# adthoms/dcora

Hardware: AMD Instinct MI355X
Metric: RBCD iterations/sec, sphere2500 5-agent split (higher is better)
Workload: dtype f64

## Files before the change

dcora_amd/capi.py:

```python
import ctypes as C
import os
import subprocess

import numpy as np

_HERE = os.path.dirname(os.path.abspath(__file__))
LIB_PATH = os.path.join(_HERE, "lib", "libdcora_hip.so")
HEADER_PATH = os.path.join(os.path.dirname(_HERE), "include", "dcora_hip.h")


class DcoraError(RuntimeError):
    def __init__(self, status, msg):
        super().__init__("dcora status %d: %s" % (status, msg))
        self.status = status


class Dims(C.Structure):
    _fields_ = [("r", C.c_int), ("d", C.c_int), ("n", C.c_int), ("l", C.c_int), ("b", C.c_int), ("layout", C.c_int)]


LAYOUT_AUTO, LAYOUT_SE, LAYOUT_RA = 0, 1, 2


class ROptParams(C.Structure):
# ... 167 lines not shown
    "dcora_exchange_create_ra": (C.c_int, [_vp, C.c_char_p, C.POINTER(_vp)]),
    "dcora_exchange_info": (C.c_int, [_vp, _dp]),
    "dcora_exchange_link_report": (C.c_int, [_vp, _dp]),
    "dcora_exchange_post": (C.c_int, [_vp, _ip, C.c_int]),
    "dcora_exchange_wait": (C.c_int, [_vp, _ip, C.c_int]),
    "dcora_exchange_evaluate": (C.c_int, [_vp, _PD, _PD, _vp, _PI]),
    "dcora_exchange_rbcd_iterate": (C.c_int, [_vp, C.c_int, _PD, _PD, _vp, _PI]),
    "dcora_exchange_rbcd_tick": (C.c_int, [_vp, _ip, C.c_int, C.c_int]),
    "dcora_exchange_run_coloured": (C.c_int, [_vp, C.c_int, C.c_double, _PI, _vp, _vp]),
    "dcora_exchange_set_X": (C.c_int, [_vp, _dp]),
    "dcora_exchange_gather_X": (C.c_int, [_vp, _dp]),
    "dcora_exchange_barrier": (C.c_int, [_vp]),
    "dcora_exchange_all_ready": (C.c_int, [_vp, C.c_int, _PI]),
    "dcora_exchange_update_weights": (C.c_int, [_vp, C.c_int, _vp]),
    "dcora_exchange_set_weights": (C.c_int, [_vp, _dp]),
    "dcora_exchange_get_weights": (C.c_int, [_vp, _dp]),
    "dcora_exchange_certify": (C.c_int, [_vp, C.c_int, _vp, _vp, _vp, C.c_double, _PI, _PD, _PD, _dp,
                                         C.POINTER(C.c_longlong), _PI]),
    "dcora_exchange_host_selftest": (C.c_int, [C.c_char_p, C.c_int, C.c_int, C.c_int, C.c_int, _PD]),
    "dcora_exchange_host_selftest_team": (C.c_int, [C.c_char_p, C.c_int, C.c_int, C.c_int, C.c_int, C.c_int, _PD]),
    "dcora_exchange_team_enable": (C.c_int, [_vp, C.POINTER(TeamParams)]),
    "dcora_exchange_agent_status": (C.c_int, [_vp, C.c_int, C.POINTER(AgentStatus), _PI]),
    "dcora_exchange_loop_closure_stats": (C.c_int, [_vp, C.c_int, _ip]),
    "dcora_exchange_should_terminate": (C.c_int, [_vp, _PI]),
    "dcora_exchange_should_update_weights": (C.c_int, [_vp, _PI]),
    "dcora_exchange_team_info": (C.c_int, [_vp, _ip]),
    "dcora_exchange_run_team": (C.c_int, [_vp, _PI, _vp, _vp, _vp, _vp, _PI, _PI]),
    "dcora_debug_exchange_leave_stale": (C.c_int, [C.c_char_p, C.c_int, C.c_int]),
    "dcora_debug_exchange_probe_fault": (C.c_int, [C.c_int]),
    "dcora_cert_prepare": (C.c_int, [C.POINTER(Dims), _ip, _ip, C.c_int, C.c_int]),
    "dcora_debug_tcg_run_fault": (C.c_int, [C.c_int]),
    "dcora_debug_tcg_run_fault_at": (C.c_int, [C.c_int, C.c_int]),
    "dcora_debug_wg_sums": (C.c_int, [C.c_int, _dp, _dp]),
    "dcora_problem_solver_info": (C.c_int, [_vp, _dp]),
    "dcora_ra_rbcd_create": (C.c_int, [_vp, C.POINTER(RbcdOptions), C.POINTER(_vp)]),
    "dcora_ra_rbcd_destroy": (C.c_int, [_vp]),
    "dcora_ra_rbcd_info": (C.c_int, [_vp, _PI, _vp]),
    "dcora_ra_rbcd_set_X": (C.c_int, [_vp, _dp]),
    "dcora_ra_rbcd_get_X": (C.c_int, [_vp, _dp]),
    "dcora_ra_rbcd_certify": (C.c_int, [_vp, C.c_double, _PI, _PD, _PD, _vp, C.POINTER(C.c_longlong), _vp]),
    "dcora_ra_rbcd_iterate": (C.c_int, [_vp, C.c_int, _PD, _PD, _vp, _PI]),
    "dcora_ra_rbcd_evaluate": (C.c_int, [_vp, _PD, _PD, _vp, _PI]),
    "dcora_ra_rbcd_run": (C.c_int, [_vp, C.c_int, C.c_double, _PI, _vp, _vp, _vp]),
    "dcora_ra_rbcd_iterate_set": (C.c_int, [_vp, _ip, C.c_int, C.c_int]),
    "dcora_ra_rbcd_set_acceleration": (C.c_int, [_vp, C.c_int]),
    "dcora_ra_rbcd_agent_colours": (C.c_int, [_vp, _ip, _PI]),
    "dcora_ra_rbcd_run_coloured": (C.c_int, [_vp, C.c_int, C.c_double, _PI, _vp, _vp]),
    "dcora_ra_rbcd_last_result": (C.c_int, [_vp, C.POINTER(ROptResult)]),
    "dcora_problem_time_qapply": (C.c_int, [_vp, C.c_int, _PD, _PD]),
    "dcora_problem_time_qapply_rotating": (C.c_int, [C.POINTER(_vp), C.c_int, C.c_int, _PD]),
    "dcora_problem_qapply_info": (C.c_int, [_vp, _dp]),
    "dcora_problem_time_precond": (C.c_int, [_vp, C.c_int, _PD, _PD]),
    "dcora_problem_precond_info": (C.c_int, [_vp, _dp]),
    "dcora_precond_cache_info": (C.c_int, [_dp]),
    "dcora_precond_cache_clear": (C.c_int, []),
    "dcora_robust_params_default": (None, [C.POINTER(RobustParams)]),
    "dcora_robust_weights": (C.c_int, [C.POINTER(RobustParams), C.c_int, C.c_int, _dp, _dp]),
    "dcora_chi2inv": (C.c_int, [C.c_double, C.c_int, _PD]),
    "dcora_robust_error_threshold_at_quantile": (C.c_int, [C.c_double, C.c_int, _PD]),
    "dcora_robust_single_rotation_averaging": (C.c_int, [C.c_int, C.c_int, _dp, _vp, C.c_double, _dp, _ip]),
    "dcora_robust_single_pose_averaging": (C.c_int, [C.c_int, C.c_int, _dp, _dp, _vp, _vp, C.c_double, _dp, _dp, _ip]),
    "dcora_agent_neighbor_transforms": (C.c_int, [C.c_int, C.c_int, _ip, _dp, _dp, _dp, _dp, _dp]),
    "dcora_agent_robust_neighbor_transform": (C.c_int, [C.c_int, C.c_int, _dp, C.c_int, C.c_int, _dp, _PI, _PI]),
    "dcora_log_trajectory": (C.c_int, [C.c_char_p, C.c_int, C.c_int, _dp]),
    "dcora_fixed_stiefel_variable": (C.c_int, [C.c_int, C.c_int, _dp]),
    "dcora_agent_initialize_in_global_frame": (C.c_int, [C.POINTER(Dims), _dp, _dp, _dp, _dp]),
# ... 49 lines not shown
```

dcora_amd/csrc/capi.hip:

```cpp
#include <cstdio>
#include <cstring>
#include <new>

#include "../../include/dcora_hip.h"
#include "cert.h"
#include "device_chol.h"
#include "device_problem.h"
#include "host_graph.h"
#include "host_threads.h"
#include "ra_rbcd.h"
#include "rbcd.h"
#include "precond_cache.h"
#include "exchange.h"
#include "host_robust.h"
#include "robust.h"
#include "round.h"

namespace dcora {
const std::string &get_last_error();
}
using namespace dcora;

struct dcora_problem_s {
  DeviceProblem p;
// ... 249 lines not shown
  });
}

int dcora_problem_solver_info(dcora_problem_t p, double *info) {
  return abi_call({p, info}, [&]() -> int {
    const DeviceProblem &P = p->p;
    info[0] = !P.use_pc() ? 0 : (P.tcg_run_ok ? 2 : 1);
    return DCORA_OK;
  });
}
int dcora_debug_tcg_run_fault(int runs) {
  g_tcg_run_fault_skip.store(0);
  g_tcg_run_fault.store(runs < 0 ? 0 : runs);
  return DCORA_OK;
}
int dcora_debug_tcg_run_fault_at(int skip, int runs) {
  g_tcg_run_fault_skip.store(skip < 0 ? 0 : skip);
  g_tcg_run_fault.store(runs < 0 ? 0 : runs);
  return DCORA_OK;
}
int dcora_debug_wg_sums(int nv, const double *in, double *out) {
  return abi_call({in, out}, [&]() -> int {
    if (no_device()) return DCORA_ERR_NO_DEVICE;
    if (nv != 33 && nv != 41 && nv != 49) return bad("dcora_debug_wg_sums: nv is 33, 41 or 49 (8 r + 1 at r = 4, 5, 6)");
    const size_t nin = (size_t)nv * 256, nout = (size_t)2 * nv * 17;
    DevBuf<double> I, O;
    DCORA_HIP(I.alloc(nin));
    DCORA_HIP(O.alloc(nout));
    DCORA_HIP(hipMemcpy(I.p, in, nin * sizeof(double), hipMemcpyHostToDevice));
    DCORA_HIP(hipMemset(O.p, 0, nout * sizeof(double)));
    if (launch_debug_wg_sums(nullptr, nv, I.p, O.p) < 0) return bad("dcora_debug_wg_sums: the launch failed");
    DCORA_HIP(hipDeviceSynchronize());
    DCORA_HIP(hipMemcpy(out, O.p, nout * sizeof(double), hipMemcpyDeviceToHost));
    return DCORA_OK;
  });
}
int dcora_problem_time_precond(dcora_problem_t p, int reps, double *avg_ms, double *bytes) {
  return abi_call({p, avg_ms, bytes}, [&] { return p->p.time_precond(reps, avg_ms, bytes); });
}
int dcora_problem_precond_info(dcora_problem_t p, double *info) {
  return abi_call({p, info}, [&]() -> int {
    const DeviceProblem &P = p->p;
    info[0] = !P.has_precond ? 0 : (P.sparse_precond ? 2 : 1);
    info[1] = !P.has_precond ? 0 : (P.sparse_precond ? P.sp.launches() : 1);
    info[2] = (double)P.precond_nnzL;
    info[3] = P.precond_setup_ms;
    info[4] = !P.has_precond ? 0 : (P.sparse_precond ? P.sp.weights_per_apply : (double)P.m.k * P.m.k);
    return DCORA_OK;
  });
}

int dcora_debug_sparse_weights_digest(dcora_problem_t p, double *out4) {
  return abi_call({p, out4}, [&]() -> int {
    const DeviceProblem &P = p->p;
    if (!P.sparse_precond || !P.sp.im) return bad("the problem has no sparse preconditioner");
    const DevBuf<double> &v = P.sp.im->vals;
    std::vector<double> h(v.n);
    DCORA_HIP(hipSetDevice(P.device));
    DCORA_HIP(hipMemcpy(h.data(), v.p, v.n * sizeof(double), hipMemcpyDeviceToHost));
    long double s0 = 0, s1 = 0, s2 = 0;
    for (size_t i = 0; i < h.size(); ++i) {
      s0 += h[i];
      s1 += std::fabs(h[i]);
      s2 += h[i] * (double)(i % 97 + 1);
    }
    out4[0] = (double)h.size();
// ... 1551 lines not shown
```

dcora_amd/csrc/fused_run.hip:

```cpp
#include <algorithm>
#include <atomic>
#include <cstdio>

#include "kernels.h"
#include "tcg_rules.h"
#include "pose_group.h"
#include "fused_pc.h"

namespace dcora {

namespace {

__device__ __forceinline__ int wg_sums_logical_lane(int p) { return ((p >> 5) & 1) | ((p >> 3) & 2) | ((p & 15) << 2); }
template <bool HALF32>
__device__ __forceinline__ double wg_sums_swap_add(double x, double y) {
  typedef unsigned u2 __attribute__((ext_vector_type(2)));
  u2 lo, hi;
  if constexpr (HALF32) {
    lo = __builtin_amdgcn_permlane32_swap((unsigned)__double2loint(x), (unsigned)__double2loint(y), false, false);
    hi = __builtin_amdgcn_permlane32_swap((unsigned)__double2hiint(x), (unsigned)__double2hiint(y), false, false);
  } else {
    lo = __builtin_amdgcn_permlane16_swap((unsigned)__double2loint(x), (unsigned)__double2loint(y), false, false);
    hi = __builtin_amdgcn_permlane16_swap((unsigned)__double2hiint(x), (unsigned)__double2hiint(y), false, false);
  }
  return __hiloint2double((int)hi[0], (int)lo[0]) + __hiloint2double((int)hi[1], (int)lo[1]);
}
template <int NV>
__device__ __forceinline__ void wg_row_sums(const double (&v)[NV], double (*sP)[4 * kPcNW], int wave, int lane) {
  constexpr int N1 = (NV + 1) / 2, N2 = (N1 + 1) / 2;
  double a[N1], b[N2];
#pragma unroll
  for (int j = 0; j < N1; ++j) a[j] = wg_sums_swap_add<true>(v[2 * j], 2 * j + 1 < NV ? v[2 * j + 1] : 0.0);
#pragma unroll
  for (int j = 0; j < N2; ++j) {
    double s = wg_sums_swap_add<false>(a[2 * j], 2 * j + 1 < N1 ? a[2 * j + 1] : 0.0);
    s += dpp_move<0xB1>(s);
    s += dpp_move<0x4E>(s);
    b[j] = s;
  }
  if ((lane & 3) == 0) {
    const int sub = ((lane >> 3) & 2) | (lane >> 5), slot = wave * 4 + ((lane >> 2) & 3);
#pragma unroll
    for (int j = 0; j < N2; ++j)
      if (4 * j + sub < NV) sP[4 * j + sub][slot] = b[j];
  }
}

constexpr int kRunShards = 32, kRunCopies = 64, kRunStride = 32;
constexpr int kRunSyncWords = (kRunShards + 1 + kRunCopies + 1) * kRunStride;
constexpr int kRunQCap = 1024;
struct TcgRunArgs {
  ManiDesc m;
  int ldm;
  const double *Minv;
  CsrDev Q;
  Buf2 grad, X, S;
  double *d0, *d1, *Hd, *eta, *Heta, *z, *p1r, *p3, *pC;
  unsigned *sync;
  SolverCtl *ctl;
  HostFlags *hf;
  int seq, pbA;
  int fault;
#ifdef DCORA_RUN_STAMPS
  long long *stamps;
#endif
};
#ifdef DCORA_RUN_STAMPS
#define RUN_STAMP(i)                                                            \
  do {                                                                          \
    __builtin_amdgcn_sched_barrier(0);                                          \
    if (a.stamps && blockIdx.x == 0 && threadIdx.x == 0 && (i) < 64) a.stamps[(i)] = wall_clock64(); \
    __builtin_amdgcn_sched_barrier(0);                                          \
  } while (0)
#else
#define RUN_STAMP(i) \
  do {                \
  } while (0)
#endif
constexpr int kRunStamp0 = 4, kRunStampsPerIter = 10;
__device__ __forceinline__ double ld_coh(const double *p) {
  return __hip_atomic_load(p, __ATOMIC_RELAXED, __HIP_MEMORY_SCOPE_AGENT);
}
__device__ __forceinline__ void st_coh(double *p, double v) {
  __hip_atomic_store(p, v, __ATOMIC_RELAXED, __HIP_MEMORY_SCOPE_AGENT);
}
__device__ __forceinline__ double2 pc_ld16_coh(__amdgpu_buffer_rsrc_t rs, unsigned voff, unsigned soff) {
  const pc_v4u v = __builtin_amdgcn_raw_buffer_load_b128(rs, voff, soff, 16);
  return __builtin_bit_cast(double2, v);
}
constexpr unsigned kRunAbortBit = 0x80000000u;
__device__ __forceinline__ bool run_grid_step(unsigned *sync, unsigned step, int *s_ok) {
  __builtin_amdgcn_s_waitcnt(0);
  __syncthreads();
  if (threadIdx.x == 0) {
    unsigned *shard = sync, *top = sync + kRunShards * kRunStride, *done = top + kRunStride,
             *abort_w = done + kRunCopies * kRunStride;
    const int i = blockIdx.x, G = gridDim.x, sh = i % kRunShards;
    const unsigned in_shard = (unsigned)((G - sh + kRunShards - 1) / kRunShards), want = step + 1;
    const unsigned shards_used = (unsigned)(G < kRunShards ? G : kRunShards);
    const unsigned a = __hip_atomic_fetch_add(shard + sh * kRunStride, 1u, __ATOMIC_RELAXED, __HIP_MEMORY_SCOPE_AGENT);
    if (a + 1 == want * in_shard) {
      const unsigned b = __hip_atomic_fetch_add(top, 1u, __ATOMIC_RELAXED, __HIP_MEMORY_SCOPE_AGENT);
      if (!(b & kRunAbortBit) && b + 1 == want * shards_used)
        for (int c = 0; c < kRunCopies; ++c)
          __hip_atomic_store(done + c * kRunStride, want, __ATOMIC_RELAXED, __HIP_MEMORY_SCOPE_AGENT);
    }
    long long t0 = wall_clock64();
    const unsigned *p = done + (i % kRunCopies) * kRunStride;
    int ok = 1;
    unsigned spins = 0;
    while (__hip_atomic_load(p, __ATOMIC_RELAXED, __HIP_MEMORY_SCOPE_AGENT) < want) {
      __builtin_amdgcn_s_sleep(1);
      if ((++spins & 63u) == 0) {
        if (__hip_atomic_load(abort_w, __ATOMIC_RELAXED, __HIP_MEMORY_SCOPE_AGENT) != 0u) {
          ok = 0;
          break;
        }
        if (wall_clock64() - t0 > 200000) {
          unsigned cur = __hip_atomic_load(top, __ATOMIC_RELAXED, __HIP_MEMORY_SCOPE_AGENT);
          bool gave_up = false;
          for (;;) {
            if (cur & kRunAbortBit) {
              gave_up = true;
              break;
            }
            if (cur >= want * shards_used) break;
            if (__hip_atomic_compare_exchange_strong(top, &cur, cur | kRunAbortBit, __ATOMIC_RELAXED, __ATOMIC_RELAXED,
                                                     __HIP_MEMORY_SCOPE_AGENT)) {
              gave_up = true;
              break;
            }
          }
          if (gave_up) {
            __hip_atomic_store(abort_w, 1u, __ATOMIC_RELAXED, __HIP_MEMORY_SCOPE_AGENT);
            ok = 0;
            break;
          }
          t0 = wall_clock64();
        }
      }
    }
    *s_ok = ok;
  }
  __syncthreads();
  return *s_ok != 0;
}

template <int D, int R, int NS>
__global__ __launch_bounds__(kPcBlock) void k_tcg_run(TcgRunArgs a) {
  constexpr int DH = D + 1, PB = 2, NR = PB * DH, RM = R;
  extern __shared__ __align__(16) double s_img[];
  double *const s_res = s_img;
  __shared__ double s_P[NR * RM + 1][4 * kPcNW];
  __shared__ double s_Z[NR * RM + 1], s_R[NR * RM], s_W[NR * RM], s_D[NR * RM], s_H[NR * RM];
  __shared__ double s_red[16];
  __shared__ int s_ci[kRunQCap];
  __shared__ double s_v[kRunQCap];
  __shared__ int s_ok;
  SolverCtl *ctl = a.ctl;
  const int seq = a.seq;
  RUN_STAMP(0);
  const int st_o = ctl->outer_done_stamp, cur = ctl->cur & 1;
  if (seq > st_o) return;
  const double c_Delta = ctl->Delta, c_ngf = ctl->ngf;
  const int c_max_inner = ctl->max_inner;
  const ManiDesc m = a.m;
  constexpr int r = R;
  const int k = m.k, ldm = a.ldm;
  const int pose0 = blockIdx.x * PB;
  const int npose = min(PB, m.n - pose0);
  const int j0 = pose0 * DH, nrow = npose * DH;
  const int wave = threadIdx.x >> 6, lane = threadIdx.x & 63;
  const int wave_u = __builtin_amdgcn_readfirstlane(wave);
  const int e = threadIdx.x;
  const bool own = e < nrow * r;
  const size_t oown = (size_t)j0 * r + e;
  const int lc = e / r, t = e - lc * r;
  const int g = threadIdx.x >> 3, tt = threadIdx.x & (GW - 1);
  const bool pact = (g < npose) && (tt < r);
  const size_t o = (size_t)(pose0 + min(g, npose - 1)) * DH * r;
  const double *__restrict__ grad = a.grad.p[cur];
  const double *__restrict__ X = a.X.p[cur];
  const unsigned vec_bytes = (unsigned)((size_t)r * k * sizeof(double));
  const __amdgpu_buffer_rsrc_t rs_g = __builtin_amdgcn_make_buffer_rsrc(const_cast<double *>(grad), 0, vec_bytes, 0x00020000);
  const __amdgpu_buffer_rsrc_t rs_h = __builtin_amdgcn_make_buffer_rsrc(a.Hd, 0, vec_bytes, 0x00020000);
// ... 18 lines not shown
  for (int i = threadIdx.x; i < pend - pbeg; i += kPcBlock) {
    s_ci[i] = a.Q.ci[pbeg + i];
    s_v[i] = a.Q.v[pbeg + i];
  }
  const int myb = own ? a.Q.rp[j0 + lc] - pbeg : 0, mye = own ? a.Q.rp[j0 + lc + 1] - pbeg : 0;
  Row<D> Y;
  ld_row<D>(X + o, r, tt, pact, Y);
  double S[D][D];
  {
    const double *__restrict__ Sblk = a.S.p[cur];
#pragma unroll
    for (int aa = 0; aa < D; ++aa)
#pragma unroll
      for (int b = 0; b < D; ++b) S[aa][b] = (g < npose) ? Sblk[(size_t)(pose0 + g) * D * D + aa + b * D] : 0.0;
  }
  double o_r = own ? grad[oown] : 0.0, o_eta = 0, o_Heta = 0, o_d = 0, o_h = 0;
  const int cpad = ((k + 127) / 128) * 128;
  const long Nc = (long)k * r;
  const int npair = (int)((Nc + 1) >> 1);
  const int nstep = cpad / 128;
  double zr = 0, dPd = 0, ePe = 0, ePd = 0, alpha = 0, ePen = 0;
  const double n0 = c_ngf;
  int status = TR_MAXITER, iters_done = 0;
  unsigned gstep = 0;
  double acc[NR * RM + 1];
  double nrm2 = 0;
  auto product = [&](int sb) {
#pragma unroll
    for (int i = 0; i < NR * RM; ++i) acc[i] = 0;
#pragma unroll
    for (int u = 0; u < NS; ++u) {
      const int sidx = wave_u + kPcNW * u;
      if (sidx < nstep) {
        const double2 *__restrict__ xs = reinterpret_cast<const double2 *>(s_img) + (size_t)(sidx * 64 + llane) * r;
        double x[2 * RM];
#pragma unroll
        for (int tq = 0; tq < RM; ++tq) {
          const double2 xx = xs[tq];
          x[2 * tq] = xx.x;
          x[2 * tq + 1] = xx.y;
        }
#pragma unroll
        for (int tq = 0; tq < RM; ++tq)
#pragma unroll
          for (int q = 0; q < NR; ++q)
            acc[q * RM + tq] = fma(x[tq], mreg[u][q].x, fma(x[r + tq], mreg[u][q].y, acc[q * RM + tq]));
      }
    }
    RUN_STAMP(sb);
#ifdef DCORA_RUN_BUTTERFLY_SUMS
    acc[NR * RM] = nrm2;
#pragma unroll
    for (int i = 0; i <= NR * RM; ++i) {
      const double v = row16_sum_dpp(acc[i]);
      if ((lane & 15) == 0) s_P[i][wave * 4 + (lane >> 4)] = v;
    }
#else
    acc[NR * RM] = __shfl(nrm2, llane);
    wg_row_sums<NR * RM + 1>(acc, s_P, wave, lane);
#endif
    RUN_STAMP(sb + 1);
    __syncthreads();
    if ((int)threadIdx.x <= NR * RM) {
      double v = 0;
#pragma unroll
      for (int w = 0; w < 4 * kPcNW; ++w) v += s_P[threadIdx.x][w];
      s_Z[threadIdx.x] = v;
// ... 40 lines not shown
      const double gr = grad[oown];
      a0 = o_eta * gr;
      a1 = o_eta * o_Heta;
      s_R[lc * RM + t] = o_eta;
    }
    __syncthreads();
    if (wave == 0) {
      Row<D> Yn = Y;
#pragma unroll
      for (int aa = 0; aa < DH; ++aa) Yn.e[aa] += 1.0 * (pact ? s_R[(g * DH + aa) * RM + tt] : 0.0);
      row_qf<D>(Yn);
      st_row<D>(a.X.p[cur ^ 1] + o, r, tt, pact, Yn);
    }
    const double t0 = block_sum(a0, s_red);
    const double t1 = block_sum(a1, s_red);
    if (threadIdx.x == 0) {
      a.pC[2 * blockIdx.x] = t0;
      a.pC[2 * blockIdx.x + 1] = t1;
    }
  };
  auto give_up = [&]() {
    if (threadIdx.x == 0) {
      ctl->outer_done_stamp = seq - 1;
      host_store(&a.hf->tcg_abort_seq, seq);
    }
  };
#pragma unroll
  for (int u = 0; u < kPcSB; ++u) {
    const int i = u * kPcBlock + (int)threadIdx.x;
    if (i < npair) {
      const double2 x = xg[u];
      nrm2 = fma(x.x, x.x, nrm2);
      nrm2 = fma(x.y, x.y, nrm2);
      reinterpret_cast<double2 *>(s_res)[i] = x;
    }
  }
  for (long i = 2L * npair + threadIdx.x; i < (long)cpad * r; i += kPcBlock) s_res[i] = 0.0;
  if (own) s_R[lc * RM + t] = o_r;
  __syncthreads();
  RUN_STAMP(1);
  product(64);
  project_z();
  RUN_STAMP(2);
  if (c_max_inner <= 0) {
    status = TR_MAXITER;
    finish();
    return;
  }
  if (a.fault && blockIdx.x == 0) return;
  if (!run_grid_step(a.sync, gstep++, &s_ok)) return give_up();
  RUN_STAMP(3);
  for (int iter = 0;; ++iter) {
    const int par = iter & 1;
    [[maybe_unused]] const int sb0 = kRunStamp0 + kRunStampsPerIter * iter;
    double *__restrict__ d_new = par ? a.d1 : a.d0;
    const double *__restrict__ d_old = par ? a.d0 : a.d1;
    {
      constexpr int kRunGB = 24;
      double ga[kRunGB], gz[kRunGB];
      double z_own = 0;
      if (own) {
        z_own = ld_coh(a.z + oown);
#pragma unroll
        for (int q = 0; q < kRunGB; ++q) {
          const bool ok = myb + q < mye;
          const size_t oo = ok ? (size_t)s_ci[myb + q] * r + t : 0;
          gz[q] = ld_coh(a.z + oo);
          ga[q] = (iter > 0) ? ld_coh(d_old + oo) : 0.0;
        }
      }
// ... 32 lines not shown
          }
#pragma unroll
          for (int q = 0; q < 8; ++q) accw += w8[q] * (beta * a8[q] - b8[q]);
        }
        dn = (iter > 0) ? beta * o_d - z_own : -z_own;
        st_coh(d_new + oown, dn);
        o_d = dn;
        s_W[e] = accw;
        s_D[e] = dn;
      }
      __syncthreads();
      if (wave == 0) {
        Row<D> V, W;
#pragma unroll
        for (int aa = 0; aa < DH; ++aa) {
          W.e[aa] = pact ? s_W[(g * DH + aa) * r + tt] : 0.0;
          V.e[aa] = pact ? s_D[(g * DH + aa) * r + tt] : 0.0;
        }
        row_sub_AS<D>(W, V, S);
        row_tangent<D>(Y, W);
        if (pact)
#pragma unroll
          for (int aa = 0; aa < DH; ++aa) {
            st_coh(a.Hd + o + aa * r + tt, W.e[aa]);
            s_H[(g * DH + aa) * r + tt] = W.e[aa];
          }
        double dacc = 0;
#pragma unroll
        for (int aa = 0; aa < DH; ++aa) dacc += V.e[aa] * W.e[aa];
        if (!pact) dacc = 0;
        const double rs = row16_sum_dpp(dacc);
        if (lane == 0) st_coh(a.p1r + blockIdx.x, rs);
      }
      __syncthreads();
      if (own) o_h = s_H[e];
    }
    RUN_STAMP(sb0 + 1);
    if (!run_grid_step(a.sync, gstep++, &s_ok)) return give_up();
    RUN_STAMP(sb0 + 2);
    double2 xh[kPcSB];
#pragma unroll
    for (int u = 0; u < kPcSB; ++u) xh[u] = pc_ld16_coh(rs_h, voff_t, (unsigned)u * kPcBlock * 16u);
    double d_Hd;
    {
      const int rows_per = a.pbA / 2, nrows = gridDim.x, nblk = (nrows + rows_per - 1) / rows_per;
      double part = 0;
      if (lane < nblk) {
        const int b0 = lane * rows_per;
        double wsum[4] = {0, 0, 0, 0};
#pragma unroll
        for (int w = 0; w < 4; ++w) {
          double rs4[4];
#pragma unroll
          for (int q = 0; q < 4; ++q) {
            const int ri = w * 4 + q;
            rs4[q] = (ri < rows_per && b0 + ri < nrows) ? ld_coh(a.p1r + b0 + ri) : 0.0;
          }
          wsum[w] = (rs4[0] + rs4[1]) + (rs4[2] + rs4[3]);
        }
        double tsum = 0;
#pragma unroll
        for (int w = 0; w < 4; ++w) tsum += wsum[w];
        part = tsum;
      }
      d_Hd = wave_sum(part);
    }
    const double c_zr = zr, c_dPd = dPd, c_ePe = ePe, c_ePd = ePd;
    alpha = tcg_alpha(c_zr, d_Hd);
    const double e_Pe_new = tcg_e_Pe_new(alpha, c_dPd, c_ePe, c_ePd);
    const bool boundary = tcg_boundary(d_Hd, e_Pe_new, c_Delta);
    const double step = boundary ? tcg_tau(c_dPd, c_ePe, c_ePd, c_Delta) : alpha;
    ePen = e_Pe_new;
    if (own) {
      o_eta = o_eta + step * o_d;
      o_Heta = o_Heta + step * o_h;
    }
    if (boundary) {
      status = tcg_boundary_status(d_Hd);
      iters_done = iter + 1;
      finish();
      return;
    }
    if (own) {
      const double rr = fma(alpha, o_h, o_r);
      o_r = rr;
      s_R[lc * RM + t] = rr;
    }
    RUN_STAMP(sb0 + 3);
    nrm2 = 0;
#pragma unroll
    for (int u = 0; u < kPcSB; ++u) {
      const int i = u * kPcBlock + (int)threadIdx.x;
      if (i < npair) {
        double2 x = reinterpret_cast<double2 *>(s_res)[i];
        x.x = fma(alpha, xh[u].x, x.x);
        x.y = fma(alpha, xh[u].y, x.y);
        nrm2 = fma(x.x, x.x, nrm2);
        nrm2 = fma(x.y, x.y, nrm2);
        reinterpret_cast<double2 *>(s_res)[i] = x;
      }
    }
    __syncthreads();
    RUN_STAMP(sb0 + 4);
    product(sb0 + 5);
    {
      if (tcg_residual_done(sqrt(s_Z[NR * RM]), n0)) {
        status = tcg_residual_status(n0);
        iters_done = iter + 1;
        finish();
        return;
      }
    }
    project_z();
    if (iter + 1 >= c_max_inner) {
      iters_done = iter + 1;
      finish();
      return;
    }
    RUN_STAMP(sb0 + 8);
    if (!run_grid_step(a.sync, gstep++, &s_ok)) return give_up();
    RUN_STAMP(sb0 + 9);
  }
}

template <int NV>
__global__ __launch_bounds__(kPcBlock) void k_debug_wg_sums(const double *__restrict__ in, double *__restrict__ out) {
  __shared__ double s_P[NV][4 * kPcNW];
  const int wave = threadIdx.x >> 6, lane = threadIdx.x & 63;
  double v[NV];
#pragma unroll
  for (int form = 0; form < 2; ++form) {
    const int src = wave * 64 + (form == 0 ? wg_sums_logical_lane(lane) : lane);
#pragma unroll
    for (int i = 0; i < NV; ++i) v[i] = in[(size_t)i * kPcBlock + src];
    if (form == 0) {
      wg_row_sums<NV>(v, s_P, wave, lane);
    } else {
#pragma unroll
      for (int i = 0; i < NV; ++i) {
        const double s = row16_sum_dpp(v[i]);
        if ((lane & 15) == 0) s_P[i][wave * 4 + (lane >> 4)] = s;
      }
    }
    __syncthreads();
    double *__restrict__ o = out + (size_t)form * NV * (4 * kPcNW + 1);
    if ((int)threadIdx.x < NV) {
      double t = 0;
#pragma unroll
      for (int w = 0; w < 4 * kPcNW; ++w) {
        t += s_P[threadIdx.x][w];
        o[threadIdx.x * 4 * kPcNW + w] = s_P[threadIdx.x][w];
      }
      o[NV * 4 * kPcNW + threadIdx.x] = t;
    }
    __syncthreads();
  }
}

}

constexpr int kRunNS = 4;
int tcg_run_sync_words() { return kRunSyncWords; }
std::atomic<int> g_tcg_run_fault{0};
std::atomic<int> g_tcg_run_fault_skip{0};
int tcg_run_max_rows_nnz(const ManiDesc &m, const int *rp) {
  const int dh = m.d + 1;
  int worst = 0;
  for (int p0 = 0; p0 < m.n; p0 += 2) {
    const int j0 = p0 * dh, j1 = std::min(m.n, p0 + 2) * dh;
    worst = std::max(worst, rp[j1] - rp[j0]);
  }
  return worst;
}
bool tcg_run_supported(const ManiDesc &m, int ldm, int cus, int max_rows_nnz) {
  if (!m.se || m.d != 3 || m.r < 4 || m.r > 6) return false;
  if (fused_pb(m.r, m.d + 1) % 2 != 0) return false;
  if (!fused_pc_preferred(m, ldm) || fused_pc_pb(m) != 2) return false;
  const int grid = (m.n + 1) / 2;
  if (grid > cus || grid > 256) return false;
  if (m.k > kRunNS * kPcNW * 128) return false;
  const int rows_per = fused_pb(m.r, m.d + 1) / 2;
  if ((grid + rows_per - 1) / rows_per > 64) return false;
  return max_rows_nnz <= kRunQCap;
}
template <int R>
static int tcg_run_launch(hipStream_t st, const TcgRunArgs &a) {
  static LdsGrant grant;
  const int cpad = ((a.m.k + 127) / 128) * 128;
  const size_t lds = (size_t)cpad * R * sizeof(double);
  if (!grant.granted(reinterpret_cast<const void *>(&k_tcg_run<3, R, kRunNS>), lds, 40 * 1024)) return -1;
  const int grid = (a.m.n + 1) / 2;
  hipLaunchKernelGGL((k_tcg_run<3, R, kRunNS>), dim3(grid), dim3(kPcBlock), lds, st, a);
  if (hipGetLastError() != hipSuccess) return -1;
  return grid;
}
int launch_tcg_run(hipStream_t st, const TcgOperands &o, int seq) {
  count_launch();
  int fault = 0;
  bool skipped = false;
  for (int sk = g_tcg_run_fault_skip.load(); sk > 0;)
    if (g_tcg_run_fault_skip.compare_exchange_weak(sk, sk - 1)) {
      skipped = true;
      break;
    }
  for (int left = skipped ? 0 : g_tcg_run_fault.load(); left > 0;)
    if (g_tcg_run_fault.compare_exchange_weak(left, left - 1)) {
      fault = 1;
      break;
    }
  const ManiDesc &m = o.m;
  TcgRunArgs a{m, o.ldm, o.Minv, o.Q, o.grad, o.X, o.S, o.d[0], o.d[1], o.Hd, o.eta, o.Heta, o.z, o.p1, o.p3, o.pC,
               o.sync, o.ctl, o.hf, seq, fused_pb(m.r, m.d + 1), fault};
#ifdef DCORA_RUN_STAMPS
  {
    static long long *buf = nullptr;
    if (!buf) (void)hipHostMalloc((void **)&buf, 64 * sizeof(long long), hipHostMallocMapped);
    static int count = 0;
    if (buf && count > 0) {
      static double acc[64];
      static int n = 0;
      long long s0 = buf[0];
      constexpr int kShown = kRunStamp0 + 4 * kRunStampsPerIter;
      if (buf[3] > s0 && buf[kShown - 1] > 0) {
        for (int i = 0; i < kShown; ++i) acc[i] += (double)(buf[i] - s0) * 0.01;
        ++n;
      }
      for (int i = 0; i < 64; ++i) buf[i] = 0;
      if (n == 500) {
        fprintf(stderr, "k_tcg_run stamps (us from start, workgroup 0, mean of %d runs that went past their fourth iteration):", n);
        for (int i = 0; i < kShown; ++i) fprintf(stderr, " %.2f", acc[i] / n);
        fprintf(stderr, "\n");
        n = -1000000;
      }
    }
    ++count;
    a.stamps = buf;
  }
#endif
  if (m.r == 4) return tcg_run_launch<4>(st, a);
  if (m.r == 5) return tcg_run_launch<5>(st, a);
  if (m.r == 6) return tcg_run_launch<6>(st, a);
  return -1;
}
int launch_debug_wg_sums(hipStream_t st, int nv, const double *in, double *out) {
  if (nv == 33) hipLaunchKernelGGL((k_debug_wg_sums<33>), dim3(1), dim3(kPcBlock), 0, st, in, out);
  else if (nv == 41) hipLaunchKernelGGL((k_debug_wg_sums<41>), dim3(1), dim3(kPcBlock), 0, st, in, out);
  else if (nv == 49) hipLaunchKernelGGL((k_debug_wg_sums<49>), dim3(1), dim3(kPcBlock), 0, st, in, out);
  else return -1;
  return hipGetLastError() == hipSuccess ? 0 : -1;
}

}
```

dcora_amd/csrc/kernels.h:

```cpp
#pragma once
#include <hip/hip_runtime.h>

#include <atomic>
#include <climits>
#include <vector>

#include "exchange_slots.h"

namespace dcora {

constexpr int kMaxPartials = 1024;
constexpr int kBsrMaxGrid = 4096;
constexpr int kBlock = 256;
constexpr int kSpmmTile = 1536;

enum class Factor : int { Stiefel, Sphere, Euclid };
struct ManiItem {
  Factor kind;
  int col;
  int idx;
};
struct ManiDesc {
  int r, d, n, l, b, k, se;
  __host__ __device__ int rot_col(int i) const { return se ? i * (d + 1) : i * d; }
// ... 174 lines not shown
int fused_pose_blocks(const ManiDesc &m);
int fused_nsplit(const ManiDesc &m);
int fused_precond_grid(const ManiDesc &m);
int fused_update_grid(const ManiDesc &m);
struct TcgOperands {
  ManiDesc m{};
  int ldm = 0;
  const double *Minv = nullptr;
  CsrDev Q;
  BsrDev Qb;
  bool has_bsr = false;
  Buf2 grad{}, X{}, S{};
  double *d[2] = {nullptr, nullptr}, *r[2] = {nullptr, nullptr};
  double *Hd = nullptr, *eta = nullptr, *Heta = nullptr, *z = nullptr;
  double *Zpart = nullptr;
  double *W = nullptr;
  double *p1 = nullptr, *p2 = nullptr, *p3 = nullptr, *pC = nullptr;
  SolverCtl *ctl = nullptr;
  HostFlags *hf = nullptr;
  SpFold sf;
  unsigned *sync = nullptr;
  double *res_new(int iter, int first) const { return first ? r[0] : r[(iter & 1) ^ 1]; }
};
int launch_fused_hess(hipStream_t st, const TcgOperands &o, int seq, int iter, int np3);
void launch_fused_precond(hipStream_t st, const TcgOperands &o, int seq, int iter, int first, int np1);
int fused_pc_blocks(const ManiDesc &m);
bool tcg_run_supported(const ManiDesc &m, int ldm, int cus, int max_rows_nnz);
int tcg_run_sync_words();
extern std::atomic<int> g_tcg_run_fault;
extern std::atomic<int> g_tcg_run_fault_skip;
int tcg_run_max_rows_nnz(const ManiDesc &m, const int *rowptr);
int launch_tcg_run(hipStream_t st, const TcgOperands &o, int seq);
int launch_debug_wg_sums(hipStream_t st, int nv, const double *in, double *out);
bool fused_pc_preferred(const ManiDesc &m, int ldm);
bool fused_pc_ready(const ManiDesc &m, int ldm);
int launch_fused_pc(hipStream_t st, const TcgOperands &o, int seq, int iter, int first, int np1, bool retract);
enum class FinishZ {
  slices,
  keep_raw,
  from_raw
};
void launch_fused_finish(hipStream_t st, const TcgOperands &o, int seq, int iter, int first, int np2,
                         FinishZ zsrc = FinishZ::slices);
int launch_fused_grad_bsr(hipStream_t st, int r, int d, const BsrDev &A, Buf2 X, const double *G, Buf2 EG, Buf2 RG, Buf2 S,
                          int sel, double *pA, double *pB, double *posenorm, Gate g,
                          const int *agent_start = nullptr, int agents = 0, int *wg_per_agent = nullptr);
int launch_fused_grad(hipStream_t st, const ManiDesc &m, const CsrDev &Q, Buf2 X, const double *G, Buf2 EG, Buf2 RG,
                      Buf2 Sblk, int sel, double *pA, double *pB, double *posenorm, Gate g,
                      const GradRide *ride = nullptr);
int launch_g_rgrad(hipStream_t st, const ManiDesc &m, Buf2 X, Buf2 EG, Buf2 RG, Buf2 Sblk, int sel, double *partials,
                   double *posenorm, Gate g);
void launch_ctl_init(hipStream_t st, SolverCtl *c, double tol, double Delta, double maxDelta, int max_outer,
                     int stop_on_accept, int max_inner);
void launch_eval_finish(hipStream_t st, int R, const int *pose_start, const double *posenorm, const double *pA,
                        int npA, EvalOut *out_dev, int seq, double *split_scratch = nullptr, int nposes = 0,
                        const double *agent_partials = nullptr, int wg_per_agent = 0);
int eval_split_doubles();
struct RelChangeSet {
  int count;
  int agent[kMaxAgents];
};
void launch_rel_change(hipStream_t st, int r, int d, const double *X, const double *XPrev, const int *pose_start,
                       const RelChangeSet &set, double *out);
struct RelChangePublish {
  ShmStatus *slots;
  int R;
// ... 81 lines not shown
```

dcora_amd/csrc/pose_group.h:

```cpp
#pragma once
#include "kernels.h"

namespace dcora {

namespace {

constexpr int GW = 8;

__device__ __forceinline__ double f_partial4_load(const double *__restrict__ p, int np) {
  const int l = (int)(threadIdx.x & 63u);
  const double a = (l < np) ? p[l] : 0.0, b = (l + 64 < np) ? p[l + 64] : 0.0;
  const double c = (l + 128 < np) ? p[l + 128] : 0.0, d = (l + 192 < np) ? p[l + 192] : 0.0;
  return (a + b) + (c + d);
}
__device__ __forceinline__ int f_partial_index(int np) { return np <= 64 ? (int)(threadIdx.x & 63u) : (int)threadIdx.x; }
__device__ __forceinline__ double f_partial_total(double v, int np, double *sm) {
  return np <= 64 ? wave_sum(v) : block_sum(v, sm);
}
__device__ __forceinline__ double grp_sum(double v) {
  asm volatile("" : "+v"(v));
  v += dpp_move<0xB1>(v);
  asm volatile("" : "+v"(v));
  v += dpp_move<0x4E>(v);
  asm volatile("" : "+v"(v));
// ... 159 lines not shown
          B.e[p] = cs * x - sn * y;
          B.e[q] = sn * x + cs * y;
#pragma unroll
          for (int i = 0; i < D; ++i) {
            const double vx = Vm[p][i], vy = Vm[q][i];
            Vm[p][i] = cs * vx - sn * vy;
            Vm[q][i] = sn * vx + cs * vy;
          }
        }
      }
    settled = settled || off < 1e-15;
    if (__all(settled)) break;
  }
  double u[D];
#pragma unroll
  for (int j = 0; j < D; ++j) {
    const double nn = grp_sum(B.e[j] * B.e[j]);
    u[j] = B.e[j] * (nn > 0 ? 1.0 / sqrt(nn) : 0.0);
  }
  if (jacobi)
#pragma unroll
    for (int c = 0; c < D; ++c) {
      double s = 0;
#pragma unroll
      for (int j = 0; j < D; ++j) s += u[j] * Vm[j][c];
      A.e[c] = s;
    }
}

constexpr int kHessTile = 1536;
constexpr int kPosesPerBlock = kBlock / GW;
constexpr int kBsrTile = 160;

__host__ __device__ inline int fused_pb(int r, int dh) {
  const int pb = kBlock / (dh * r);
  return pb > kPosesPerBlock ? kPosesPerBlock : pb;
}

#define DCORA_LAUNCH_D(KERNEL, d, grid, st, ...)                                                 \
  do {                                                                                           \
    if ((d) == 3) hipLaunchKernelGGL(KERNEL<3>, dim3(grid), dim3(kBlock), 0, st, __VA_ARGS__);   \
    else hipLaunchKernelGGL(KERNEL<2>, dim3(grid), dim3(kBlock), 0, st, __VA_ARGS__);            \
  } while (0)

}

}
```

include/dcora_hip.h:

```cpp
#ifndef DCORA_HIP_H_
#define DCORA_HIP_H_

#ifdef __cplusplus
extern "C" {
#endif

typedef enum {
  DCORA_OK = 0,
  DCORA_ERR_BAD_ARG = 1,
  DCORA_ERR_NO_DEVICE = 2,
  DCORA_ERR_HIP = 3,
  DCORA_ERR_NOT_PD = 4,
  DCORA_ERR_NO_CONVERGENCE = 5,
  DCORA_ERR_NO_PRECONDITIONER = 6,
  DCORA_ERR_IO = 7,
  DCORA_ERR_UNSUPPORTED = 8,
  DCORA_ERR_EXCHANGE_LINK = 9
} dcora_status;

const char *dcora_status_string(int status);
const char *dcora_last_error(void);
int dcora_device_count(void);

enum {
// ... 14 lines not shown
  int method;
  int verbose;
  double gradnorm_tol;
  double RGD_stepsize;
  int RGD_use_preconditioner;
  int RTR_iterations;
  int RTR_tCG_iterations;
  double RTR_initial_radius;
} dcora_ropt_params;
void dcora_ropt_params_default(dcora_ropt_params *p);

typedef struct {
  int success;
  double fInit, gradNormInit, fOpt, gradNormOpt, elapsedMs;
  int tCGStatus;
  int outer_iterations, inner_iterations, accepted_steps;
} dcora_ropt_result;

typedef struct dcora_problem_s *dcora_problem_t;

int dcora_problem_create(const dcora_dims *dims, const int *rowptr, const int *colidx, const double *vals,
                         const double *G, double precond_reg, int device, dcora_problem_t *out);
int dcora_problem_destroy(dcora_problem_t p);
int dcora_problem_set_linear_term(dcora_problem_t p, const double *G);
int dcora_problem_cost(dcora_problem_t p, const double *X, double *f);
int dcora_problem_eucgrad(dcora_problem_t p, const double *X, double *out);
int dcora_problem_riegrad(dcora_problem_t p, const double *X, double *out, double *norm);
int dcora_problem_hessvec(dcora_problem_t p, const double *X, const double *V, double *out);
int dcora_debug_hessvec_solver_form(dcora_problem_t p, const double *X, const double *V, double *out, double *dots);
int dcora_problem_solver_info(dcora_problem_t p, double *info);
int dcora_debug_tcg_run_fault(int runs);
int dcora_debug_tcg_run_fault_at(int skip, int runs);
int dcora_debug_wg_sums(int nv, const double *in, double *out);
int dcora_problem_precondition(dcora_problem_t p, const double *X, const double *V, double *out);
int dcora_problem_retract(dcora_problem_t p, const double *X, const double *V, double *out);
int dcora_problem_tangent_project(dcora_problem_t p, const double *X, const double *V, double *out);
int dcora_problem_escape_saddle(dcora_problem_t p, const double *Xopt, double theta, const double *v,
                                double gradient_tolerance, double preconditioned_gradient_tolerance,
                                int is_second_order, double *Xout, int *success);
int dcora_manifold_project(const dcora_dims *dims, const double *M, double *out, int device);

int dcora_optimizer_optimize(dcora_problem_t p, const dcora_ropt_params *params, const double *X0, double *Xout,
                             dcora_ropt_result *result);

typedef struct dcora_csr_s *dcora_csr_t;
int dcora_csr_info(dcora_csr_t m, int *n, int *nnz);
int dcora_csr_copy(dcora_csr_t m, int *rowptr, int *colidx, double *vals);
int dcora_csr_destroy(dcora_csr_t m);

int dcora_cert_dual_matrix(const dcora_dims *dims, const double *X, const int *rowptr, const int *colidx,
                           const double *vals, int device, dcora_csr_t *S);
int dcora_cert_is_psd(int k, const int *rowptr, const int *colidx, const double *vals, int block, int *is_psd);
int dcora_cert_is_psd_device(int k, const int *rowptr, const int *colidx, const double *vals, int block, int device,
                             int *is_psd, double *info8);
int dcora_chol_host_selftest(int k, const int *rowptr, const int *colidx, const double *vals, int block, int *is_pd,
                             double *resid, double *info4);
int dcora_chol_cache_clear(void);
int dcora_cert_min_eig(int k, const int *rowptr, const int *colidx, const double *vals, int max_iterations,
                       double min_eig_num_tol, int num_lanczos_vectors, unsigned long long seed, int device,
                       double *lambda_min, double *v, long *num_matvecs);
int dcora_cert_fast_verification(int k, const int *rowptr, const int *colidx, const double *vals, double eta,
                                 int block, int device, int *is_psd, double *theta, double *x, double *lambda_min);

int dcora_cert_suboptimality_gap(const dcora_dims *dims, const double *X, double lambda_lower_bound, double *gap,
                                 double *n_eff);
int dcora_cert_lambda_min_certified(int k, const int *rowptr, const int *colidx, const double *vals, double eta,
// ... 241 lines not shown
```

Baseline: 4634.

## Parallelise grid-barrier done broadcast and hoist row-sum loads ahead of image loads

The grid barrier now has all 64 lanes of wave 0 write the done-word copies in parallel, replacing a serial loop in thread 0. After the barrier, the per-block row-sum loads are issued up front with a compile-time rows_per, then a trimmed set of image pieces is loaded. A block-wide __syncthreads before the barrier is removed. The residual update is restructured into grouped loads, FMA and stores behind scheduling barriers, with a padded image layout and a debug API that exposes it. The aim is to shorten barrier latency and expose more memory-level parallelism, at the cost of added complexity and register pressure.

```diff
diff --git a/dcora_amd/capi.py b/dcora_amd/capi.py
--- a/dcora_amd/capi.py
+++ b/dcora_amd/capi.py
@@ -223,6 +223,7 @@
     "dcora_debug_tcg_run_fault": (C.c_int, [C.c_int]),
     "dcora_debug_tcg_run_fault_at": (C.c_int, [C.c_int, C.c_int]),
     "dcora_debug_wg_sums": (C.c_int, [C.c_int, _dp, _dp]),
+    "dcora_debug_run_image": (C.c_int, [C.c_int, C.c_int, _ip, _ip, _PI]),
     "dcora_problem_solver_info": (C.c_int, [_vp, _dp]),
     "dcora_ra_rbcd_create": (C.c_int, [_vp, C.POINTER(RbcdOptions), C.POINTER(_vp)]),
     "dcora_ra_rbcd_destroy": (C.c_int, [_vp]),
diff --git a/dcora_amd/csrc/capi.hip b/dcora_amd/csrc/capi.hip
--- a/dcora_amd/csrc/capi.hip
+++ b/dcora_amd/csrc/capi.hip
@@ -305,6 +305,14 @@
     if (launch_debug_wg_sums(nullptr, nv, I.p, O.p) < 0) return bad("dcora_debug_wg_sums: the launch failed");
     DCORA_HIP(hipDeviceSynchronize());
     DCORA_HIP(hipMemcpy(out, O.p, nout * sizeof(double), hipMemcpyDeviceToHost));
+    return DCORA_OK;
+  });
+}
+int dcora_debug_run_image(int r, int k, int *off, int *lanes, int *bytes) {
+  return abi_call({off, lanes, bytes}, [&]() -> int {
+    const int b = tcg_run_image_map(r, k, off, lanes);
+    if (b < 0) return bad("dcora_debug_run_image: r is 4, 5 or 6 and 1 <= k <= 2048");
+    *bytes = b;
     return DCORA_OK;
   });
 }
diff --git a/dcora_amd/csrc/fused_run.hip b/dcora_amd/csrc/fused_run.hip
--- a/dcora_amd/csrc/fused_run.hip
+++ b/dcora_amd/csrc/fused_run.hip
@@ -11,7 +11,7 @@
 
 namespace {
 
-__device__ __forceinline__ int wg_sums_logical_lane(int p) { return ((p >> 5) & 1) | ((p >> 3) & 2) | ((p & 15) << 2); }
+__host__ __device__ __forceinline__ int wg_sums_logical_lane(int p) { return ((p >> 5) & 1) | ((p >> 3) & 2) | ((p & 15) << 2); }
 template <bool HALF32>
 __device__ __forceinline__ double wg_sums_swap_add(double x, double y) {
   typedef unsigned u2 __attribute__((ext_vector_type(2)));
@@ -49,6 +49,9 @@
 constexpr int kRunShards = 32, kRunCopies = 64, kRunStride = 32;
 constexpr int kRunSyncWords = (kRunShards + 1 + kRunCopies + 1) * kRunStride;
 constexpr int kRunQCap = 1024;
+constexpr int kRunNS = 4;
+__host__ __device__ constexpr int run_img_off(int i) { return 16 * i; }
+constexpr size_t run_img_bytes(int r, int cpad) { return (size_t)run_img_off(cpad * r / 2) + 16; }
 struct TcgRunArgs {
   ManiDesc m;
   int ldm;
@@ -59,7 +62,7 @@
   unsigned *sync;
   SolverCtl *ctl;
   HostFlags *hf;
-  int seq, pbA;
+  int seq;
   int fault;
 #ifdef DCORA_RUN_STAMPS
   long long *stamps;
@@ -92,19 +95,27 @@
 __device__ __forceinline__ bool run_grid_step(unsigned *sync, unsigned step, int *s_ok) {
   __builtin_amdgcn_s_waitcnt(0);
   __syncthreads();
-  if (threadIdx.x == 0) {
-    unsigned *shard = sync, *top = sync + kRunShards * kRunStride, *done = top + kRunStride,
-             *abort_w = done + kRunCopies * kRunStride;
+  static_assert(kRunCopies == 64, "one copy of the done word per lane of wave 0");
+  if (threadIdx.x < 64) {
+    unsigned *shard = sync, *top = sync + kRunShards * kRunStride, *done = top + kRunStride;
     const int i = blockIdx.x, G = gridDim.x, sh = i % kRunShards;
     const unsigned in_shard = (unsigned)((G - sh + kRunShards - 1) / kRunShards), want = step + 1;
     const unsigned shards_used = (unsigned)(G < kRunShards ? G : kRunShards);
-    const unsigned a = __hip_atomic_fetch_add(shard + sh * kRunStride, 1u, __ATOMIC_RELAXED, __HIP_MEMORY_SCOPE_AGENT);
-    if (a + 1 == want * in_shard) {
-      const unsigned b = __hip_atomic_fetch_add(top, 1u, __ATOMIC_RELAXED, __HIP_MEMORY_SCOPE_AGENT);
-      if (!(b & kRunAbortBit) && b + 1 == want * shards_used)
-        for (int c = 0; c < kRunCopies; ++c)
-          __hip_atomic_store(done + c * kRunStride, want, __ATOMIC_RELAXED, __HIP_MEMORY_SCOPE_AGENT);
-    }
+    int last = 0;
+    if (threadIdx.x == 0) {
+      const unsigned a = __hip_atomic_fetch_add(shard + sh * kRunStride, 1u, __ATOMIC_RELAXED, __HIP_MEMORY_SCOPE_AGENT);
+      if (a + 1 == want * in_shard) {
+        const unsigned b = __hip_atomic_fetch_add(top, 1u, __ATOMIC_RELAXED, __HIP_MEMORY_SCOPE_AGENT);
+        last = !(b & kRunAbortBit) && b + 1 == want * shards_used;
+      }
+    }
+    if (__builtin_amdgcn_readfirstlane(last))
+      __hip_atomic_store(done + threadIdx.x * kRunStride, want, __ATOMIC_RELAXED, __HIP_MEMORY_SCOPE_AGENT);
+  }
+  if (threadIdx.x == 0) {
+    unsigned *top = sync + kRunShards * kRunStride, *done = top + kRunStride, *abort_w = done + kRunCopies * kRunStride;
+    const int i = blockIdx.x, G = gridDim.x;
+    const unsigned want = step + 1, shards_used = (unsigned)(G < kRunShards ? G : kRunShards);
     long long t0 = wall_clock64();
     const unsigned *p = done + (i % kRunCopies) * kRunStride;
     int ok = 1;
@@ -149,8 +160,11 @@
 template <int D, int R, int NS>
 __global__ __launch_bounds__(kPcBlock) void k_tcg_run(TcgRunArgs a) {
   constexpr int DH = D + 1, PB = 2, NR = PB * DH, RM = R;
+  constexpr int kImgGroup = R == 6 ? 1 : 4;
+  constexpr int kImgPieces = kImgGroup == 1 ? kPcSB : NS * kPcNW * 128 * R / 2 / kPcBlock;
+  static_assert(kImgPieces <= kPcSB && kImgPieces % kImgGroup == 0, "the image's pieces come in whole groups");
   extern __shared__ __align__(16) double s_img[];
-  double *const s_res = s_img;
+  auto img_pair = [&](int i) { return reinterpret_cast<double2 *>(s_img) + run_img_off(i) / 16; };
   __shared__ double s_P[NR * RM + 1][4 * kPcNW];
   __shared__ double s_Z[NR * RM + 1], s_R[NR * RM], s_W[NR * RM], s_D[NR * RM], s_H[NR * RM];
   __shared__ double s_red[16];
@@ -235,7 +249,7 @@
     for (int u = 0; u < NS; ++u) {
       const int sidx = wave_u + kPcNW * u;
       if (sidx < nstep) {
-        const double2 *__restrict__ xs = reinterpret_cast<const double2 *>(s_img) + (size_t)(sidx * 64 + llane) * r;
+        const double2 *__restrict__ xs = img_pair((sidx * 64 + llane) * r);
         double x[2 * RM];
 #pragma unroll
         for (int tq = 0; tq < RM; ++tq) {
@@ -342,10 +356,10 @@
       const double2 x = xg[u];
       nrm2 = fma(x.x, x.x, nrm2);
       nrm2 = fma(x.y, x.y, nrm2);
-      reinterpret_cast<double2 *>(s_res)[i] = x;
-    }
-  }
-  for (long i = 2L * npair + threadIdx.x; i < (long)cpad * r; i += kPcBlock) s_res[i] = 0.0;
+      *img_pair(i) = x;
+    }
+  }
+  for (int i = npair + (int)threadIdx.x; i < cpad * r / 2; i += kPcBlock) *img_pair(i) = double2{0.0, 0.0};
   if (own) s_R[lc * RM + t] = o_r;
   __syncthreads();
   RUN_STAMP(1);
@@ -444,32 +458,32 @@
         const double rs = row16_sum_dpp(dacc);
         if (lane == 0) st_coh(a.p1r + blockIdx.x, rs);
       }
-      __syncthreads();
-      if (own) o_h = s_H[e];
     }
     RUN_STAMP(sb0 + 1);
     if (!run_grid_step(a.sync, gstep++, &s_ok)) return give_up();
     RUN_STAMP(sb0 + 2);
-    double2 xh[kPcSB];
-#pragma unroll
-    for (int u = 0; u < kPcSB; ++u) xh[u] = pc_ld16_coh(rs_h, voff_t, (unsigned)u * kPcBlock * 16u);
+    constexpr int rows_per = fused_pb(R, DH) / 2;
+    static_assert(rows_per <= 8, "the row sums of one k_fused_hess workgroup are loaded as 8 values");
+    const int nrows = gridDim.x, nblk = (nrows + rows_per - 1) / rows_per;
+    double rs16[16];
+    {
+      const int b0 = min(lane, nblk - 1) * rows_per;
+#pragma unroll
+      for (int ri = 0; ri < 16; ++ri) rs16[ri] = (ri < rows_per && b0 + ri < nrows) ? ld_coh(a.p1r + b0 + ri) : 0.0;
+    }
+    __builtin_amdgcn_sched_barrier(0);
+    double2 xh[kImgPieces];
+#pragma unroll
+    for (int u = 0; u < kImgPieces; ++u) xh[u] = pc_ld16_coh(rs_h, voff_t, (unsigned)u * kPcBlock * 16u);
+    __builtin_amdgcn_sched_barrier(0);
+    if (own) o_h = s_H[e];
     double d_Hd;
     {
-      const int rows_per = a.pbA / 2, nrows = gridDim.x, nblk = (nrows + rows_per - 1) / rows_per;
       double part = 0;
       if (lane < nblk) {
-        const int b0 = lane * rows_per;
-        double wsum[4] = {0, 0, 0, 0};
-#pragma unroll
-        for (int w = 0; w < 4; ++w) {
-          double rs4[4];
-#pragma unroll
-          for (int q = 0; q < 4; ++q) {
-            const int ri = w * 4 + q;
-            rs4[q] = (ri < rows_per && b0 + ri < nrows) ? ld_coh(a.p1r + b0 + ri) : 0.0;
-          }
-          wsum[w] = (rs4[0] + rs4[1]) + (rs4[2] + rs4[3]);
-        }
+        double wsum[4];
+#pragma unroll
+        for (int w = 0; w < 4; ++w) wsum[w] = (rs16[4 * w] + rs16[4 * w + 1]) + (rs16[4 * w + 2] + rs16[4 * w + 3]);
         double tsum = 0;
 #pragma unroll
         for (int w = 0; w < 4; ++w) tsum += wsum[w];
@@ -500,16 +514,42 @@
     }
     RUN_STAMP(sb0 + 3);
     nrm2 = 0;
-#pragma unroll
-    for (int u = 0; u < kPcSB; ++u) {
-      const int i = u * kPcBlock + (int)threadIdx.x;
-      if (i < npair) {
-        double2 x = reinterpret_cast<double2 *>(s_res)[i];
-        x.x = fma(alpha, xh[u].x, x.x);
-        x.y = fma(alpha, xh[u].y, x.y);
-        nrm2 = fma(x.x, x.x, nrm2);
-        nrm2 = fma(x.y, x.y, nrm2);
-        reinterpret_cast<double2 *>(s_res)[i] = x;
+    if constexpr (kImgGroup == 1) {
+#pragma unroll
+      for (int u = 0; u < kImgPieces; ++u) {
+        const int i = u * kPcBlock + (int)threadIdx.x;
+        if (i < npair) {
+          double2 x = *img_pair(i);
+          x.x = fma(alpha, xh[u].x, x.x);
+          x.y = fma(alpha, xh[u].y, x.y);
+          nrm2 = fma(x.x, x.x, nrm2);
+          nrm2 = fma(x.y, x.y, nrm2);
+          *img_pair(i) = x;
+        }
+      }
+    } else {
+#pragma unroll
+      for (int u0 = 0; u0 < kImgPieces; u0 += kImgGroup) {
+        if (u0 * kPcBlock < npair) {
+          double2 *pp[kImgGroup];
+          double2 x[kImgGroup];
+#pragma unroll
+          for (int j = 0; j < kImgGroup; ++j) {
+            const int i = (u0 + j) * kPcBlock + (int)threadIdx.x;
+            pp[j] = i < npair ? img_pair(i) : img_pair(cpad * r / 2);
+            x[j] = *pp[j];
+          }
+          __builtin_amdgcn_sched_barrier(0);
+#pragma unroll
+          for (int j = 0; j < kImgGroup; ++j) {
+            x[j].x = fma(alpha, xh[u0 + j].x, x[j].x);
+            x[j].y = fma(alpha, xh[u0 + j].y, x[j].y);
+            const double n2 = fma(x[j].y, x[j].y, fma(x[j].x, x[j].x, nrm2));
+            nrm2 = (u0 + j) * kPcBlock + (int)threadIdx.x < npair ? n2 : nrm2;
+          }
+#pragma unroll
+          for (int j = 0; j < kImgGroup; ++j) *pp[j] = x[j];
+        }
       }
     }
     __syncthreads();
@@ -571,7 +611,6 @@
 
 }
 
-constexpr int kRunNS = 4;
 int tcg_run_sync_words() { return kRunSyncWords; }
 std::atomic<int> g_tcg_run_fault{0};
 std::atomic<int> g_tcg_run_fault_skip{0};
@@ -599,7 +638,7 @@
 static int tcg_run_launch(hipStream_t st, const TcgRunArgs &a) {
   static LdsGrant grant;
   const int cpad = ((a.m.k + 127) / 128) * 128;
-  const size_t lds = (size_t)cpad * R * sizeof(double);
+  const size_t lds = run_img_bytes(R, cpad);
   if (!grant.granted(reinterpret_cast<const void *>(&k_tcg_run<3, R, kRunNS>), lds, 40 * 1024)) return -1;
   const int grid = (a.m.n + 1) / 2;
   hipLaunchKernelGGL((k_tcg_run<3, R, kRunNS>), dim3(grid), dim3(kPcBlock), lds, st, a);
@@ -622,7 +661,7 @@
     }
   const ManiDesc &m = o.m;
   TcgRunArgs a{m, o.ldm, o.Minv, o.Q, o.grad, o.X, o.S, o.d[0], o.d[1], o.Hd, o.eta, o.Heta, o.z, o.p1, o.p3, o.pC,
-               o.sync, o.ctl, o.hf, seq, fused_pb(m.r, m.d + 1), fault};
+               o.sync, o.ctl, o.hf, seq, fault};
 #ifdef DCORA_RUN_STAMPS
   {
     static long long *buf = nullptr;
@@ -661,5 +700,12 @@
   else return -1;
   return hipGetLastError() == hipSuccess ? 0 : -1;
 }
-
-}
+int tcg_run_image_map(int r, int k, int *off, int *lanes) {
+  if (r < 4 || r > 6 || k < 1 || k > kRunNS * kPcNW * 128) return -1;
+  const int cpad = ((k + 127) / 128) * 128;
+  for (int i = 0; i < cpad * r / 2; ++i) off[i] = run_img_off(i);
+  for (int p = 0; p < 64; ++p) lanes[p] = wg_sums_logical_lane(p);
+  return (int)run_img_bytes(r, cpad);
+}
+
+}
diff --git a/dcora_amd/csrc/kernels.h b/dcora_amd/csrc/kernels.h
--- a/dcora_amd/csrc/kernels.h
+++ b/dcora_amd/csrc/kernels.h
@@ -230,6 +230,7 @@
 int tcg_run_max_rows_nnz(const ManiDesc &m, const int *rowptr);
 int launch_tcg_run(hipStream_t st, const TcgOperands &o, int seq);
 int launch_debug_wg_sums(hipStream_t st, int nv, const double *in, double *out);
+int tcg_run_image_map(int r, int k, int *off, int *lanes);
 bool fused_pc_preferred(const ManiDesc &m, int ldm);
 bool fused_pc_ready(const ManiDesc &m, int ldm);
 int launch_fused_pc(hipStream_t st, const TcgOperands &o, int seq, int iter, int first, int np1, bool retract);
diff --git a/dcora_amd/csrc/pose_group.h b/dcora_amd/csrc/pose_group.h
--- a/dcora_amd/csrc/pose_group.h
+++ b/dcora_amd/csrc/pose_group.h
@@ -215,7 +215,7 @@
 constexpr int kPosesPerBlock = kBlock / GW;
 constexpr int kBsrTile = 160;
 
-__host__ __device__ inline int fused_pb(int r, int dh) {
+__host__ __device__ constexpr int fused_pb(int r, int dh) {
   const int pb = kBlock / (dh * r);
   return pb > kPosesPerBlock ? kPosesPerBlock : pb;
 }
diff --git a/include/dcora_hip.h b/include/dcora_hip.h
--- a/include/dcora_hip.h
+++ b/include/dcora_hip.h
@@ -70,6 +70,7 @@
 int dcora_debug_tcg_run_fault(int runs);
 int dcora_debug_tcg_run_fault_at(int skip, int runs);
 int dcora_debug_wg_sums(int nv, const double *in, double *out);
+int dcora_debug_run_image(int r, int k, int *off, int *lanes, int *bytes);
 int dcora_problem_precondition(dcora_problem_t p, const double *X, const double *V, double *out);
 int dcora_problem_retract(dcora_problem_t p, const double *X, const double *V, double *out);
 int dcora_problem_tangent_project(dcora_problem_t p, const double *X, const double *V, double *out);
```

Measured after the change: 4783, median of 6. +3.2%, better.
